# alshai/Big-BWT

Hardware: NVIDIA B200
Metric: pfp_parse_throughput (higher is better)
Workload: dtype u8/u32/u64 integer

## Files before the change

### big-bwt_b200/csrc/pfp_api.cu

```cuda
#include "pfp_common.cuh"
#include "pfp_stages.cuh"
#include <errno.h>
#include <fcntl.h>
#include <stdlib.h>
#include <sys/stat.h>
#include <time.h>
#include <unistd.h>

extern "C" {
int pfp_io_read_file(const char *path, int gz_ok, uint8_t **buf, uint64_t *n, char *err, size_t errlen);
int pfp_io_write_outputs(const char *path, const pfpb200_opts *opts, const pfpb200_outputs *o,
                         char *err, size_t errlen);
}

static double wall_sec() {
    struct timespec ts;
    clock_gettime(CLOCK_MONOTONIC, &ts);
    return (double)ts.tv_sec + 1e-9 * (double)ts.tv_nsec;
}

__global__ void set_u64_k(u64 *p, u64 v) { *p = v; }

__global__ void __launch_bounds__(256) first_invalid_k(const u8 *__restrict__ t, u64 n,
                                                       unsigned long long *__restrict__ first) {
// ... 16 lines not shown

int pfp_first_invalid(pfpb200_ctx *ctx, const u8 *d_text, u64 n, u64 *d_first) {
    if (n == 0) return PFPB200_OK;
    first_invalid_k<<<ctx->sm_count * 8, 256, 0, ctx->stream>>>(d_text, n,
                                                               reinterpret_cast<unsigned long long *>(d_first));
    PFP_LAUNCHED(ctx);
    return PFPB200_OK;
}

extern "C" int pfpb200_abi_version(void) { return PFPB200_ABI_VERSION; }

extern "C" const char *pfpb200_strerror(int code) {
    switch (code) {
        case PFPB200_OK: return "ok";
        case PFPB200_E_ARG: return "invalid argument";
        case PFPB200_E_IO: return "file I/O error";
        case PFPB200_E_CUDA: return "CUDA error (no usable GPU or kernel failure)";
        case PFPB200_E_NOMEM: return "out of memory";
        case PFPB200_E_LIMIT: return "algorithm limit exceeded";
        case PFPB200_E_COLLISION: return "fingerprint collision";
        case PFPB200_E_INTERNAL: return "internal error";
        default: return "unknown error";
    }
}

extern "C" uint32_t pfpb200_launch_count(const pfpb200_ctx *ctx) { return ctx ? ctx->launches : 0; }

extern "C" const char *pfpb200_last_error(const pfpb200_ctx *ctx) { return ctx ? ctx->err : ""; }

static u64 splitmix64(u64 &s) {
    u64 z = (s += 0x9E3779B97F4A7C15ULL);
    z = (z ^ (z >> 30)) * 0xBF58476D1CE4E5B9ULL;
    z = (z ^ (z >> 27)) * 0x94D049BB133111EBULL;
    return z ^ (z >> 31);
}

extern "C" int pfpb200_create(int device, pfpb200_ctx **out) {
    if (!out) return PFPB200_E_ARG;
    *out = nullptr;
    int ndev = 0;
    if (cudaGetDeviceCount(&ndev) != cudaSuccess || device < 0 || device >= ndev) {
        cudaGetLastError();
        return PFPB200_E_CUDA;
    }
    pfpb200_ctx *ctx = new (std::nothrow) pfpb200_ctx();
    if (!ctx) return PFPB200_E_NOMEM;
    ctx->device = device;
    { const char *ev = getenv("PFPB200_LEGACY_K2"); ctx->legacy_k2 = ev && atoi(ev) != 0; }
    { const char *ev = getenv("PFPB200_K1"); ctx->k1_mode = (ev && strcmp(ev, "rolling") == 0) ? 1 : (ev && strcmp(ev, "table") == 0) ? 2 : 0; }
    { const char *ev = getenv("PFPB200_TEST_WEAK_FP"); ctx->weak_fp = (ev && atoi(ev) != 0) ? 1u : 0u; }
    { const char *ev = getenv("PFPB200_NO_SCAN_ALPHA"); ctx->no_scan_alpha = ev && atoi(ev) != 0; }
    { const char *ev = getenv("PFPB200_RANK_FULL_SORT"); ctx->rank_full_sort = ev && atoi(ev) != 0; }
    { const char *ev = getenv("PFPB200_RANK_CHUNK_PASSES"); ctx->rank_chunk_passes = ev && atoi(ev) != 0; }
    { const char *ev = getenv("PFPB200_POOL_BY_WORD"); ctx->pool_by_word = ev && atoi(ev) != 0; }
    { const char *ev = getenv("PFPB200_FUSE_K3"); ctx->fuse_k3 = ev && atoi(ev) != 0; }
    { const char *ev = getenv("PFPB200_TABLE_SCALE"); if (ev && atof(ev) >= 1.2) ctx->table_scale = atof(ev); }
    { const char *ev = getenv("PFPB200_K1_MIX"); ctx->k1_mix = ev ? atoi(ev) : 0; }
    { const char *ev = getenv("PFPB200_K2_WINDOW"); ctx->k2_window = ev ? atoi(ev) : 0; }
    auto bail = [&](int code) { pfpb200_destroy(ctx); return code; };
    if (cudaSetDevice(device) != cudaSuccess) return bail(PFPB200_E_CUDA);
    cudaDeviceProp prop;
    if (cudaGetDeviceProperties(&prop, device) != cudaSuccess) return bail(PFPB200_E_CUDA);
    ctx->sm_count = prop.multiProcessorCount;
    if (cudaStreamCreateWithFlags(&ctx->own_stream, cudaStreamNonBlocking) != cudaSuccess)
        return bail(PFPB200_E_CUDA);
    ctx->stream = ctx->own_stream;
    if (cudaMalloc(&ctx->d_flags, PFP_FLAG_SLOTS * sizeof(u64)) != cudaSuccess ||
        cudaMallocHost(&ctx->h_flags, PFP_FLAG_SLOTS * sizeof(u64)) != cudaSuccess ||
        cudaMalloc(&ctx->d_keys, NH_KEY_WORDS * sizeof(u32)) != cudaSuccess ||
        cudaMalloc(&ctx->d_alpha, 8 * sizeof(u32)) != cudaSuccess)
        return bail(PFPB200_E_NOMEM);
    u32 hk[NH_KEY_WORDS];
    u64 seed = 0x5bd1e9955bd1e995ULL;
    for (u32 i = 0; i < NH_KEY_WORDS; i++) hk[i] = (u32)(splitmix64(seed) >> 32);
    if (cudaMemcpy(ctx->d_keys, hk, sizeof(hk), cudaMemcpyHostToDevice) != cudaSuccess ||
        cudaMemset(ctx->d_flags, 0, PFP_FLAG_SLOTS * sizeof(u64)) != cudaSuccess)
        return bail(PFPB200_E_CUDA);
    set_u64_k<<<1, 1, 0, ctx->stream>>>(&ctx->d_flags[15], 1);
    if (cudaGetLastError() != cudaSuccess || cudaStreamSynchronize(ctx->stream) != cudaSuccess)
        return bail(PFPB200_E_CUDA);
    if (cudaStreamCreateWithFlags(&ctx->aux_stream, cudaStreamNonBlocking) != cudaSuccess ||
        cudaEventCreateWithFlags(&ctx->ev_aux0, cudaEventDisableTiming) != cudaSuccess ||
        cudaEventCreateWithFlags(&ctx->ev_aux1, cudaEventDisableTiming) != cudaSuccess)
        return bail(PFPB200_E_CUDA);
    if (pfp_scan_init(ctx) || pfp_stream_init(ctx) || pfp_phrase_init(ctx) || pfp_prims_init(ctx) ||
        pfp_rank_init(ctx))
        return bail(PFPB200_E_CUDA);
    *out = ctx;
    return PFPB200_OK;
}

extern "C" void pfpb200_destroy(pfpb200_ctx *ctx) {
    if (!ctx) return;
    cudaSetDevice(ctx->device);
    if (ctx->stream) cudaStreamSynchronize(ctx->stream);
    pfp_release_scratch(ctx);
    pfp_release_held(ctx);
    pfp_arena_destroy(ctx);
    if (ctx->own_stream) { cudaStreamSynchronize(ctx->own_stream); cudaStreamDestroy(ctx->own_stream); }
    if (ctx->d_flags) cudaFree(ctx->d_flags);
    if (ctx->h_flags) cudaFreeHost(ctx->h_flags);
    if (ctx->d_keys) cudaFree(ctx->d_keys);
    if (ctx->dna_table) cudaFree(ctx->dna_table);
    if (ctx->iv_etab) cudaFree(ctx->iv_etab);
    if (ctx->iv_xtab) cudaFree(ctx->iv_xtab);
    if (ctx->d_alpha) cudaFree(ctx->d_alpha);
// ... 866 lines not shown
```

### big-bwt_b200/csrc/pfp_common.cuh

```cuda
#pragma once
#include <cuda_runtime.h>
#include <stdint.h>
#include <stdio.h>
#include <string.h>
#include <vector>
#include "pfp_arith.h"
#include "../../include/pfpb200.h"

typedef uint64_t u64;
typedef uint32_t u32;
typedef uint16_t u16;
typedef uint8_t u8;
typedef int64_t i64;

struct PfpBlock { char *p; size_t n; };
struct PfpArena {
    std::vector<PfpBlock> slabs;
    std::vector<PfpBlock> free_list;
    std::vector<PfpBlock> used;
    size_t in_use = 0, peak = 0, total = 0;
};

constexpr int PFP_TILE_T = 256;
constexpr int PFP_TILE_RUN = 128;
constexpr int PFP_TILE = PFP_TILE_T * PFP_TILE_RUN;
struct ScanBits {
    const uint4 *A;
    u64 q_end;
    u64 pos_bias;
    u32 ntiles;
    uint4 *mask;
    u32 *tile_cnt;
    u64 *tile_off;
    u64 total;
    u32 max_tile_cnt;
};

constexpr int PFP_IO_THREADS = 4;
constexpr size_t PFP_IO_CHUNK = (size_t)8 << 20;
struct PfpIo {
    bool ready = false;
    void *slot[PFP_IO_THREADS][2] = {{nullptr}};
    cudaEvent_t ev[PFP_IO_THREADS][2] = {{nullptr}};
    cudaStream_t stream[PFP_IO_THREADS] = {nullptr};
};

struct pfpb200_ctx {
    int device = 0;
    PfpIo io;
    PfpArena arena;
    int sm_count = 148;
    cudaStream_t own_stream = nullptr;
    cudaStream_t stream = nullptr;
    u32 launches = 0;
    int k1_mode = 0;
    u32 *d_alpha = nullptr;
    bool alpha_valid = false;
    u32 *dna_table = nullptr;
    u32 dna_w = 0, dna_p = 0;
    void *iv_etab = nullptr;
    void *iv_xtab = nullptr;
    u32 iv_w = 0, iv_p = 0, iv_cthr = 0;
    int iv_skip = 0;
    bool no_scan_alpha = false;
    bool rank_full_sort = false;
    bool rank_chunk_passes = false;
    bool pool_by_word = false;
    bool fuse_k3 = false;
    double pool_ratio = 0.0;
    bool legacy_k2 = false;
    double table_scale = 2.0;
    u32 weak_fp = 0;
    int k1_mix = 0;
    int k2_window = 0;
    double dedup_ratio = 0.0;
    char err[512] = {0};
    std::vector<void *> scratch;
    std::vector<void *> held;
    void *bp_out[3] = {nullptr, nullptr, nullptr};
    void *up_out = nullptr;
    void *pb_out[4] = {nullptr, nullptr, nullptr, nullptr};
    void *pin_buf[5] = {nullptr, nullptr, nullptr, nullptr, nullptr};
    size_t pin_cap[5] = {0, 0, 0, 0, 0};
    cudaStream_t aux_stream = nullptr;
    cudaEvent_t ev_aux0 = nullptr, ev_aux1 = nullptr;
    cudaStream_t copy_stream = nullptr;
    cudaEvent_t ev_k2 = nullptr, ev_copy = nullptr;
    bool early_copy = false;
    bool early_done = false;
    u32 *d_keys = nullptr;
    u64 *d_flags = nullptr;
    u64 *h_flags = nullptr;
    struct {
        u64 n_in = 0, d = 0, sum_len = 0;
        u32 max_len = 0;
        u32 *uid_of_entry = nullptr, *rep = nullptr, *count = nullptr, *ulen = nullptr, *uwords = nullptr;
        u64 *uoff = nullptr;
        const u32 *len_in = nullptr, *uwords_in = nullptr;
    } mg;
    struct {
        pfpb200_shard desc;
        pfpb200_opts opts;
        u64 *ends = nullptr;
        bool ends_emitted = true;
        ScanBits bits;
        u64 n_trig = 0, P = 0, d = 0;
        u32 *uid = nullptr;
        u64 *wfpa = nullptr, *wfpb = nullptr, *pool = nullptr, *uoff = nullptr, pool_words = 0;
        u32 *ulen = nullptr, *count = nullptr, *uwords = nullptr;
        u32 *route_perm = nullptr;
        u64 *route_ooff = nullptr;
        u64 route_words_to[PFPB200_MAX_RANKS] = {0}, route_pool_to[PFPB200_MAX_RANKS] = {0};
    } sh;
};

#define PFP_FLAG_SLOTS 16
#define PFP_ERRBIT_COLLISION 1ull
#define PFP_ERRBIT_LIMIT 2ull
#define PFP_ERRBIT_INTERNAL 4ull
// ... 104 lines not shown
```

### big-bwt_b200/csrc/pfp_rank.cu

```cuda
#include "pfp_common.cuh"
#include "pfp_stages.cuh"

__device__ __forceinline__ u64 bswap64(u64 v) {
    u32 lo = (u32)v, hi = (u32)(v >> 32);
    return ((u64)__byte_perm(lo, 0, 0x0123) << 32) | (u64)__byte_perm(hi, 0, 0x0123);
}

__device__ __forceinline__ u64 word_key(const u64 *__restrict__ pool, const u64 *__restrict__ uoff,
                                        const u32 *__restrict__ uwords, u32 u, u32 r) {
    return (r < uwords[u]) ? bswap64(__ldg(pool + uoff[u] + r)) : 0ull;
}

struct AlphaMap {
    u32 bits;
    u32 chars;
    u32 depth0;
    u32 pad;
    u8 lut[256];
};

constexpr u32 ALPHA_PROBE_WORDS = 3;

__global__ void alpha_presence_k(const u64 *__restrict__ pool, const u64 *__restrict__ uoff,
                                 const u32 *__restrict__ ulen, u64 d, u32 *__restrict__ gmask) {
// ... 52 lines not shown
                             const u32 *__restrict__ ulen, const u32 *__restrict__ count, u64 d,
                             const AlphaMap *__restrict__ am, u64 *__restrict__ keys, u32 *__restrict__ vals,
                             WordMeta *__restrict__ meta) {
    __shared__ u8 lut[256];
    __shared__ u32 s_bits, s_chars;
    lut[threadIdx.x & 255] = am->lut[threadIdx.x & 255];
    if (threadIdx.x == 0) { s_bits = am->bits; s_chars = am->chars; }
    __syncthreads();
    u64 u = (u64)blockIdx.x * blockDim.x + threadIdx.x;
    if (u >= d) return;
    const u32 bits = s_bits, chars = s_chars, len = ulen[u];
    const u64 off = uoff[u];
    {
        WordMeta wm;
        wm.off = off; wm.len = len; wm.count = count[u];
        meta[u] = wm;
    }
    const u32 nc = len < chars ? len : chars;
    u64 key = 0;
    u64 v = 0;
    for (u32 i = 0; i < nc; i++) {
        if ((i & 7) == 0) v = __ldg(pool + off + (i >> 3));
        u32 c = (u32)(v >> (8 * (i & 7))) & 255u;
        key |= (u64)lut[c] << (64 - bits * (i + 1));
    }
    keys[u] = key;
    vals[u] = (u32)u;
}

__global__ void rank_heads0_k(const u64 *__restrict__ ks, u64 d, const AlphaMap *__restrict__ am, u32 begin_bit,
                              u8 *__restrict__ head, u32 *__restrict__ depth) {
    u64 i = (u64)blockIdx.x * blockDim.x + threadIdx.x;
    if (i >= d) return;
    head[i] = (i == 0 || (ks[i] >> begin_bit) != (ks[i - 1] >> begin_bit)) ? 1 : 0;
    const u32 chars = (64u - begin_bit) / am->bits;
    const u32 d0 = chars / 8u;
    depth[i] = d0 < am->depth0 ? d0 : am->depth0;
}

constexpr u32 LOCAL_MAX = 2048;
constexpr u32 WARP_MAX = 32;

__global__ void groups_compact_k(const u8 *__restrict__ head, const u32 *__restrict__ hscan, u64 d,
                                 const u32 *__restrict__ nheads, u32 *__restrict__ hp,
                                 u32 *__restrict__ gid) {
    u64 i = (u64)blockIdx.x * blockDim.x + threadIdx.x;
    if (i >= d) return;
    u32 g = hscan[i] + head[i] - 1;
    gid[i] = g;
    if (head[i]) hp[g] = (u32)i;
    if (i == 0) hp[*nheads] = (u32)d;
}

__global__ void rank_active_k(const u8 *__restrict__ head, const u32 *__restrict__ gid,
                              const u32 *__restrict__ hp, u64 d, u8 *__restrict__ act,
                              u8 *__restrict__ gh) {
    u64 i = (u64)blockIdx.x * blockDim.x + threadIdx.x;
    if (i >= d) return;
    u32 g = gid[i];
    bool big = (hp[g + 1] - hp[g]) > LOCAL_MAX;
    act[i] = big ? 1 : 0;
    gh[i] = (big && head[i]) ? 1 : 0;
}

__global__ void rank_compact_k(const u8 *__restrict__ act, const u8 *__restrict__ gh,
                               const u32 *__restrict__ ascan, const u32 *__restrict__ gscan,
                               const u32 *__restrict__ ord, const u32 *__restrict__ gid,
                               const u32 *__restrict__ hp, const u32 *__restrict__ depth, u64 d,
                               const u64 *pool, const u64 *uoff, const u32 *uwords,
                               u32 *__restrict__ apos, u64 *__restrict__ keys, u32 *__restrict__ vals,
                               u32 *__restrict__ gid_of_u) {
    u64 i = (u64)blockIdx.x * blockDim.x + threadIdx.x;
    if (i >= d || !act[i]) return;
    u32 j = ascan[i];
    u32 u = ord[i];
    u32 r = depth[hp[gid[i]]];
    apos[j] = (u32)i;
    keys[j] = word_key(pool, uoff, uwords, u, r);
    vals[j] = u;
    gid_of_u[u] = gscan[i] + gh[i] - 1;
}

__global__ void rank_gidkeys_k(const u32 *__restrict__ vs, const u32 *__restrict__ gid_of_u, u64 m,
                               u64 *__restrict__ keys2) {
    u64 j = (u64)blockIdx.x * blockDim.x + threadIdx.x;
    if (j < m) keys2[j] = gid_of_u[vs[j]];
}

__global__ void rank_writeback_k(const u32 *__restrict__ apos, const u64 *__restrict__ gk,
                                 const u32 *__restrict__ vs, u64 m, const u32 *__restrict__ gid,
                                 const u32 *__restrict__ hp, const u32 *__restrict__ depth_in,
                                 const u64 *pool, const u64 *uoff, const u32 *uwords,
                                 u32 *__restrict__ ord, u8 *__restrict__ head,
                                 u32 *__restrict__ depth_out) {
    u64 j = (u64)blockIdx.x * blockDim.x + threadIdx.x;
    if (j >= m) return;
    u32 i = apos[j];
    u32 u = vs[j];
    u32 r = depth_in[hp[gid[i]]];
    ord[i] = u;
    bool newhead = false;
    if (j > 0 && gk[j] == gk[j - 1]) {
        u32 up = vs[j - 1];
        newhead = word_key(pool, uoff, uwords, u, r) != word_key(pool, uoff, uwords, up, r);
        if (newhead) head[i] = 1;
    }
    if (newhead || head[i]) depth_out[i] = r + 1;
}

__device__ __forceinline__ u32 warp_refine(const u64 *__restrict__ wptr, u32 wn, u32 lo, u32 sz, u32 r,
                                           u32 max_chunks, u64 *__restrict__ flags) {
    u64 k0 = 0, k1 = 0, k2 = 0, k3 = 0;
    u32 have = 0;
    for (;;) {
        const bool active = sz > 1;
// ... 200 lines not shown
                if (p + 1 == S.hi[cur][p]) S.tot[l] = incl[e];
            }
        }
        tie_sync<NT>();
#pragma unroll
        for (u32 e = 0; e < TIE_E; e++) {
            const u32 p = p0 + e;
            if (e < E && p < m) {
                const u32 l = S.lo[cur][p], h = S.hi[cur][p], r = S.dep[cur][p];
                u32 np = p, nlo = l, nhi = h, nr = r;
                if (h - l > 1) {
                    const u64 T = S.tot[l];
                    const u32 n0 = (u32)(T & 0xFFFFu), n1 = (u32)((T >> 16) & 0xFFFFu);
                    const u32 idx = (u32)((incl[e] >> (16 * cls[e])) & 0xFFFFu) - 1u;
                    if (cls[e] == 0) { nlo = l; nhi = l + n0; }
                    else if (cls[e] == 1) { nlo = l + n0; nhi = l + n0 + n1; nr = r + 1; }
                    else { nlo = l + n0 + n1; nhi = h; }
                    np = nlo + idx;
                }
                S.uid[cur ^ 1][np] = S.uid[cur][p];
                S.off[cur ^ 1][np] = S.off[cur][p];
                S.wn[cur ^ 1][np] = S.wn[cur][p];
                S.lo[cur ^ 1][np] = (u16)nlo;
                S.hi[cur ^ 1][np] = (u16)nhi;
                S.dep[cur ^ 1][np] = nr;
            }
        }
        tie_sync<NT>();
        cur ^= 1;
    }
    tie_sync<NT>();
    for (u32 i = t; i < m; i += NT) ord[s + i] = S.uid[cur][i];
}

template <int NT, u32 CAP>
__device__ __forceinline__ void tie_refine(TieSort<CAP> &S, u64 *sm_v, u32 *sm_f, u32 t, u32 s, u32 m, u32 r0,
                                           const u64 *pool, const u64 *uoff, const u32 *uwords, u32 max_chunks,
                                           u32 *__restrict__ ord, u64 *__restrict__ flags) {
    const u32 E = (m + NT - 1) / NT;
    if (E <= 2) tie_refine_e<NT, CAP, 2>(S, sm_v, sm_f, t, s, m, r0, pool, uoff, uwords, max_chunks, ord, flags);
    else if (E <= 4) tie_refine_e<NT, CAP, 4>(S, sm_v, sm_f, t, s, m, r0, pool, uoff, uwords, max_chunks, ord, flags);
    else tie_refine_e<NT, CAP, 8>(S, sm_v, sm_f, t, s, m, r0, pool, uoff, uwords, max_chunks, ord, flags);
}

__global__ void rank_lists_k(const u32 *__restrict__ hp, const u32 *__restrict__ nheads, u64 d,
                             u32 *__restrict__ mid_list, u32 *__restrict__ big_list,
                             u32 *__restrict__ warp_list,
                             u32 *__restrict__ counts ) {
    u64 g = (u64)blockIdx.x * blockDim.x + threadIdx.x;
    if (g >= d || g >= *nheads) return;
    const u32 s = hp[g], m = hp[g + 1] - s;
    if (m < 2) return;
    if (m <= WARP_MAX) {
        if ((s >> 5) != ((s + m - 1) >> 5)) warp_list[atomicAdd(&counts[2], 1u)] = (u32)g;
    } else if (m <= MID_MAX) mid_list[atomicAdd(&counts[0], 1u)] = (u32)g;
    else if (m <= LOCAL_MAX) big_list[atomicAdd(&counts[1], 1u)] = (u32)g;
}

__global__ void __launch_bounds__(256) rank_mid_k(const u32 *__restrict__ hp,
                                                  const u32 *__restrict__ list,
                                                  const u32 *__restrict__ count,
                                                  const u32 *__restrict__ depth,
                                                  const u64 *pool, const u64 *uoff, const u32 *uwords,
                                                  u32 max_chunks, u32 *__restrict__ ord,
                                                  u64 *__restrict__ flags) {
    extern __shared__ __align__(16) unsigned char mid_raw[];
    const u32 lane = threadIdx.x & 31, wp = threadIdx.x >> 5;
    TieSort<MID_MAX> &S = reinterpret_cast<TieSort<MID_MAX> *>(mid_raw)[wp];
    u64 *sm_v = nullptr;
    u32 *sm_f = nullptr;
    const u32 n = *count;
    for (u32 q = blockIdx.x * 8 + wp; q < n; q += gridDim.x * 8) {
        const u32 g = list[q];
        const u32 s = hp[g], m = hp[g + 1] - s;
        tie_refine<32, MID_MAX>(S, sm_v, sm_f, lane, s, m, depth[s], pool, uoff, uwords, max_chunks, ord, flags);
    }
}

constexpr u32 LCP_MAX = 256;
constexpr u32 LCP_WALK = 4;
constexpr u32 LCP_HEAD = 1u << 20;
constexpr u32 LCP_MAX_CHUNKS = LCP_HEAD - 1;

template <u32 CAP>
struct LcpSort {
    u64 kb[CAP];
    u32 ka[CAP];
    u32 uid[CAP];
    u32 off[CAP];
    u32 wn[CAP];
    u32 dep[CAP];
    u16 lo[CAP];
    u16 pay[CAP];
    unsigned long long best;
};

__device__ __forceinline__ void prefetch_l2(const void *p) { asm volatile("prefetch.global.L2 [%0];" ::"l"(p)); }

__device__ __forceinline__ bool lcp_less(u32 a0, u64 b0, u32 a1, u64 b1) { return a0 < a1 || (a0 == a1 && b0 < b1); }

__device__ __forceinline__ void lcp_cx_shfl(u32 &ka, u64 &kb, u32 &pay, u32 j, bool up, bool lower) {
    const u32 oa = __shfl_xor_sync(0xffffffffu, ka, j);
    const u64 ob = __shfl_xor_sync(0xffffffffu, kb, j);
    const u32 op = __shfl_xor_sync(0xffffffffu, pay, j);
    const bool mine_less = lcp_less(ka, kb, oa, ob);
    const bool keep = (mine_less == lower) == up;
    if (!keep && !(ka == oa && kb == ob)) { ka = oa; kb = ob; pay = op; }
}

// ... 220 lines not shown
                        const u32 c = code < LCP_HEAD ? code : 2u * LCP_HEAD - 1u - code;
                        S.dep[p] = code == LCP_HEAD ? 0u : c + 1;
                    }
                }
            }
            tie_sync<NT>();
            if (t < 32) {
                u32 carry = 0;
                for (u32 b0 = 0; b0 < m; b0 += 32) {
                    const u32 p = b0 + t;
                    const u32 sm = __ballot_sync(0xffffffffu, p < m && S.pay[p] != 0);
                    if (p < m) {
                        const u32 below = sm & (0xFFFFFFFFu >> (31 - t));
                        S.lo[p] = (u16)(below ? b0 + (31 - __clz(below)) : carry);
                    }
                    if (sm) carry = b0 + (31 - __clz(sm));
                }
            }
            tie_sync<NT>();
        }
    }
    tie_sync<NT>();
    for (u32 p = t; p < m; p += NT) ord[s + p] = S.uid[p];
}

__global__ void __launch_bounds__(256, 3) rank_lcp_k(const u32 *__restrict__ hp, const u32 *__restrict__ list,
                                                  const u32 *__restrict__ count, const u32 *__restrict__ depth,
                                                  const u64 *__restrict__ pool, const u64 *__restrict__ uoff,
                                                  const u32 *__restrict__ uwords, const u32 *__restrict__ occ_of_word,
                                                  u32 max_chunks, u32 *__restrict__ ord, u64 *__restrict__ flags) {
    extern __shared__ __align__(16) unsigned char lcp_raw[];
    const u32 lane = threadIdx.x & 31, wp = threadIdx.x >> 5;
    LcpSort<LCP_MAX> &S = reinterpret_cast<LcpSort<LCP_MAX> *>(lcp_raw)[wp];
    const u32 n = *count;
    for (u32 gq = blockIdx.x * 8 + wp; gq < n; gq += gridDim.x * 8) {
        const u32 g = list[gq];
        const u32 s = hp[g], m = hp[g + 1] - s;
        lcp_refine<32, LCP_MAX>(S, lane, s, m, depth[s], pool, uoff, uwords, occ_of_word, max_chunks, ord, flags);
    }
}

__global__ void __launch_bounds__(256) rank_lcp_cta_k(const u32 *__restrict__ hp, const u32 *__restrict__ list,
                                                      const u32 *__restrict__ count, const u32 *__restrict__ depth,
                                                      const u64 *__restrict__ pool, const u64 *__restrict__ uoff,
                                                      const u32 *__restrict__ uwords, const u32 *__restrict__ occ_of_word,
                                                      u32 max_chunks, u32 *__restrict__ ord, u64 *__restrict__ flags) {
    extern __shared__ __align__(16) unsigned char lcp_cta_raw[];
    LcpSort<LOCAL_MAX> &S = *reinterpret_cast<LcpSort<LOCAL_MAX> *>(lcp_cta_raw);
    const u32 n = *count;
    for (u32 gq = blockIdx.x; gq < n; gq += gridDim.x) {
        const u32 g = list[gq];
        const u32 s = hp[g], m = hp[g + 1] - s;
        lcp_refine<256, LOCAL_MAX>(S, threadIdx.x, s, m, depth[s], pool, uoff, uwords, occ_of_word, max_chunks, ord, flags);
    }
}

__global__ void __launch_bounds__(256) rank_cta_k(const u32 *__restrict__ hp,
                                                  const u32 *__restrict__ list,
                                                  const u32 *__restrict__ count,
                                                  const u32 *__restrict__ depth,
                                                  const u64 *pool, const u64 *uoff, const u32 *uwords,
                                                  u32 max_chunks, u32 *__restrict__ ord,
                                                  u64 *__restrict__ flags) {
    extern __shared__ __align__(16) unsigned char cta_raw[];
    TieSort<LOCAL_MAX> &S = *reinterpret_cast<TieSort<LOCAL_MAX> *>(cta_raw);
    __shared__ u64 sm_v[8];
    __shared__ u32 sm_f[8];
    const u32 n = *count;
    for (u32 q = blockIdx.x; q < n; q += gridDim.x) {
        const u32 g = list[q];
        const u32 s = hp[g], m = hp[g + 1] - s;
        tie_refine<256, LOCAL_MAX>(S, sm_v, sm_f, threadIdx.x, s, m, depth[s], pool, uoff, uwords, max_chunks, ord,
                                   flags);
    }
}

int pfp_rank_init(pfpb200_ctx *ctx) {
    PFP_CUDA(ctx, cudaFuncSetAttribute(rank_cta_k, cudaFuncAttributeMaxDynamicSharedMemorySize,
                                       (int)sizeof(TieSort<LOCAL_MAX>)));
    PFP_CUDA(ctx, cudaFuncSetAttribute(rank_mid_k, cudaFuncAttributeMaxDynamicSharedMemorySize,
                                       (int)(8 * sizeof(TieSort<MID_MAX>))));
    PFP_CUDA(ctx, cudaFuncSetAttribute(rank_lcp_k, cudaFuncAttributeMaxDynamicSharedMemorySize,
                                       (int)(8 * sizeof(LcpSort<LCP_MAX>))));
    PFP_CUDA(ctx, cudaFuncSetAttribute(rank_lcp_cta_k, cudaFuncAttributeMaxDynamicSharedMemorySize,
                                       (int)sizeof(LcpSort<LOCAL_MAX>)));
    return PFPB200_OK;
}

int pfp_rank_stage(pfpb200_ctx *ctx, DictArrays &D, u32 **order, u32 *rounds, bool alpha_from_scan) {
    const int TB = 256;
    const u64 d = D.d;
    const u32 nbd = pfp_blocks(d, TB);
    const u32 max_chunks = (D.max_len + 7) / 8 + 1;
    u64 *k0 = nullptr, *k1 = nullptr, *ks = nullptr;
    u32 *v0 = nullptr, *v1 = nullptr, *vs = nullptr;
    u32 *ord = nullptr, *depth = nullptr, *hscan = nullptr, *hp = nullptr, *gid = nullptr;
    u8 *head = nullptr;
    AlphaMap *am = nullptr;
    u32 *amask = nullptr;
    PFP_TRY(pfp_alloc_t(ctx, &k0, d));
    PFP_TRY(pfp_alloc_t(ctx, &k1, d));
    PFP_TRY(pfp_alloc_t(ctx, &v0, d));
    PFP_TRY(pfp_alloc_t(ctx, &v1, d));
    PFP_TRY(pfp_alloc_t(ctx, &ord, d));
    PFP_TRY(pfp_alloc_t(ctx, &depth, d));
    PFP_TRY(pfp_alloc_t(ctx, &hscan, d));
    PFP_TRY(pfp_alloc_t(ctx, &hp, d + 1));
    PFP_TRY(pfp_alloc_t(ctx, &gid, d));
    PFP_TRY(pfp_alloc_t(ctx, &head, d));
    PFP_TRY(pfp_alloc_t(ctx, &am, 1));
    PFP_TRY(pfp_alloc_t(ctx, &amask, 8));
    if (alpha_from_scan) {
        PFP_CUDA(ctx, cudaMemcpyAsync(amask, ctx->d_alpha, 8 * sizeof(u32), cudaMemcpyDeviceToDevice, ctx->stream));
    } else {
        PFP_CUDA(ctx, cudaMemsetAsync(amask, 0, 8 * sizeof(u32), ctx->stream));
        alpha_presence_k<<<nbd, TB, 0, ctx->stream>>>(D.pool, D.uoff, D.ulen, d, amask);
        PFP_LAUNCHED(ctx);
    }
    alpha_build_k<<<1, 32, 0, ctx->stream>>>(amask, am, alpha_from_scan ? 1 : 0);
    PFP_LAUNCHED(ctx);
    PFP_TRY(pfp_alloc_t(ctx, &D.meta, d));
    rank_keys0_k<<<nbd, TB, 0, ctx->stream>>>(D.pool, D.uoff, D.ulen, D.count, d, am, k0, v0, D.meta);
    PFP_LAUNCHED(ctx);
    int lg = 1;
    while (lg < 32 && (1ull << lg) < d) lg++;
    int sort_bits = (2 * lg + 2 + 7) / 8 * 8;
    if (sort_bits > 64 || ctx->rank_full_sort) sort_bits = 64;
    const int begin_bit = 64 - sort_bits;
    PFP_TRY(pfp_radix_sort_pairs(ctx, k0, v0, k1, v1, d, begin_bit, 64, &ks, &vs));
    rank_heads0_k<<<nbd, TB, 0, ctx->stream>>>(ks, d, am, (u32)begin_bit, head, depth);
    PFP_LAUNCHED(ctx);
    PFP_CUDA(ctx, cudaMemcpyAsync(ord, vs, d * sizeof(u32), cudaMemcpyDeviceToDevice, ctx->stream));

    u8 *act = nullptr, *gh = nullptr;
    u32 *ascan = nullptr, *gscan = nullptr, *apos = nullptr, *gid_of_u = nullptr, *depth2 = nullptr;
    u32 *d_nheads = reinterpret_cast<u32 *>(&ctx->d_flags[4]);
    u32 r = 1;
    bool big_bufs = false;
    for (;; r++) {
        PFP_CUDA(ctx, cudaMemsetAsync(&ctx->d_flags[1], 0, 4 * sizeof(u64), ctx->stream));
        PFP_TRY(pfp_exclusive_scan_u8_u32(ctx, head, hscan, d, d_nheads));
        groups_compact_k<<<nbd, TB, 0, ctx->stream>>>(head, hscan, d, d_nheads, hp, gid);
        PFP_LAUNCHED(ctx);
        if (d < 2) break;
        if (!big_bufs) {
            PFP_TRY(pfp_alloc_t(ctx, &act, d));
            PFP_TRY(pfp_alloc_t(ctx, &gh, d));
            PFP_TRY(pfp_alloc_t(ctx, &ascan, d));
            PFP_TRY(pfp_alloc_t(ctx, &gscan, d));
            big_bufs = true;
        }
        rank_active_k<<<nbd, TB, 0, ctx->stream>>>(head, gid, hp, d, act, gh);
        PFP_LAUNCHED(ctx);
        PFP_TRY(pfp_exclusive_scan_u8_u32(ctx, act, ascan, d, reinterpret_cast<u32 *>(&ctx->d_flags[1])));
        PFP_TRY(pfp_exclusive_scan_u8_u32(ctx, gh, gscan, d, reinterpret_cast<u32 *>(&ctx->d_flags[2])));
        PFP_CUDA(ctx, cudaMemcpyAsync(ctx->h_flags, ctx->d_flags, 3 * sizeof(u64),
                                      cudaMemcpyDeviceToHost, ctx->stream));
        PFP_CUDA(ctx, cudaStreamSynchronize(ctx->stream));
        u64 m = (u32)ctx->h_flags[1], ng = (u32)ctx->h_flags[2];
        if (m == 0) break;
        if (r > max_chunks + 1)
            return pfp_fail(ctx, PFPB200_E_INTERNAL,
                            "ranking did not separate %llu words after %u rounds (duplicate words?)",
                            (unsigned long long)m, r);
        if (!apos) {
            PFP_TRY(pfp_alloc_t(ctx, &apos, d));
            PFP_TRY(pfp_alloc_t(ctx, &gid_of_u, d));
            PFP_TRY(pfp_alloc_t(ctx, &depth2, d));
        }
        rank_compact_k<<<nbd, TB, 0, ctx->stream>>>(act, gh, ascan, gscan, ord, gid, hp, depth, d, D.pool,
                                                    D.uoff, D.uwords, apos, k0, v0, gid_of_u);
        PFP_LAUNCHED(ctx);
        PFP_TRY(pfp_radix_sort_pairs(ctx, k0, v0, k1, v1, m, 0, 64, &ks, &vs));
        u64 *g_in = (ks == k0) ? k1 : k0;
        u32 *v_other = (vs == v0) ? v1 : v0;
        const u32 nbm = pfp_blocks(m, TB);
        rank_gidkeys_k<<<nbm, TB, 0, ctx->stream>>>(vs, gid_of_u, m, g_in);
        PFP_LAUNCHED(ctx);
        int bits = 1;
        while (bits < 32 && (1ull << bits) < ng) bits++;
        u64 *gs = nullptr;
        u32 *vs2 = nullptr;
        PFP_TRY(pfp_radix_sort_pairs(ctx, g_in, vs, ks, v_other, m, 0, bits, &gs, &vs2));
        PFP_CUDA(ctx, cudaMemcpyAsync(depth2, depth, d * sizeof(u32), cudaMemcpyDeviceToDevice, ctx->stream));
        rank_writeback_k<<<nbm, TB, 0, ctx->stream>>>(apos, gs, vs2, m, gid, hp, depth, D.pool, D.uoff,
                                                      D.uwords, ord, head, depth2);
        PFP_LAUNCHED(ctx);
        u32 *tdp = depth; depth = depth2; depth2 = tdp;
    }
    if (d >= 2) {
        u32 *mid_list = v1, *big_list = v0;
        u32 *warp_list = reinterpret_cast<u32 *>(k1);
        u32 *counts = reinterpret_cast<u32 *>(&ctx->d_flags[5]);
        PFP_CUDA(ctx, cudaMemsetAsync(counts, 0, 4 * sizeof(u32), ctx->stream));
        rank_lists_k<<<nbd, TB, 0, ctx->stream>>>(hp, d_nheads, d, mid_list, big_list, warp_list, counts);
        PFP_LAUNCHED(ctx);
        u64 want = (d / 2 + 7) / 8;
        u64 maxb = (u64)ctx->sm_count * 16;
        u32 nbw = (u32)(want < maxb ? want : maxb);
        if (nbw == 0) nbw = 1;
        rank_window_k<<<nbw, 256, 0, ctx->stream>>>(hp, gid, depth, D.pool, D.uoff, D.uwords, d, max_chunks, 0, ord,
                                                    ctx->d_flags);
        PFP_LAUNCHED(ctx);
        rank_warp_k<<<nbw, 256, 0, ctx->stream>>>(hp, warp_list, counts + 2, depth, D.pool, D.uoff, D.uwords, max_chunks,
                                                  ord, ctx->d_flags);
        PFP_LAUNCHED(ctx);
        const bool chunk_passes = ctx->rank_chunk_passes || max_chunks >= LCP_MAX_CHUNKS;
        if (chunk_passes)
            rank_mid_k<<<ctx->sm_count * 4, 256, 8 * sizeof(TieSort<MID_MAX>), ctx->stream>>>(
                hp, mid_list, counts, depth, D.pool, D.uoff, D.uwords, max_chunks, ord, ctx->d_flags);
        else
            rank_lcp_k<<<ctx->sm_count * 6, 256, 8 * sizeof(LcpSort<LCP_MAX>), ctx->stream>>>(
                hp, mid_list, counts, depth, D.pool, D.uoff, D.uwords, D.count, max_chunks, ord, ctx->d_flags);
        PFP_LAUNCHED(ctx);
        if (chunk_passes)
            rank_cta_k<<<ctx->sm_count * 4, 256, sizeof(TieSort<LOCAL_MAX>), ctx->stream>>>(
                hp, big_list, counts + 1, depth, D.pool, D.uoff, D.uwords, max_chunks, ord, ctx->d_flags);
        else
            rank_lcp_cta_k<<<ctx->sm_count * 3, 256, sizeof(LcpSort<LOCAL_MAX>), ctx->stream>>>(
                hp, big_list, counts + 1, depth, D.pool, D.uoff, D.uwords, D.count, max_chunks, ord, ctx->d_flags);
        PFP_LAUNCHED(ctx);
        PFP_CUDA(ctx, cudaMemcpyAsync(ctx->h_flags, ctx->d_flags, sizeof(u64), cudaMemcpyDeviceToHost,
                                      ctx->stream));
        PFP_CUDA(ctx, cudaStreamSynchronize(ctx->stream));
        if (ctx->h_flags[0] & PFP_ERRBIT_INTERNAL)
            return pfp_fail(ctx, PFPB200_E_INTERNAL, "ranking found words that never differ (duplicates?)");
    }
    *rounds = r;
    *order = ord;
    void *to_free[] = {k0, k1, v0, v1, depth, depth2, hscan, hp, gid, head, am, amask, act, gh, ascan,
                       gscan, apos, gid_of_u};
    for (void *q : to_free) PFP_TRY(pfp_free_now(ctx, q));
    return PFPB200_OK;
}

__device__ __forceinline__ void out_span(const u64 *pool, u64 off, u32 len, u32 strip_w, u32 *skip,
                                         u32 *outlen) {
    *skip = 0;
    *outlen = len;
    if (strip_w) {
        u32 l = len - strip_w;
        if ((u8)(pool[off] & 0xFF) == PFP_DOLLAR) { *skip = 1; l -= 1; }
        *outlen = l;
    }
}

__global__ void dict_layout_k(const u32 *__restrict__ ord, u64 d, const DictArrays D, u32 strip_w,
                              u32 *__restrict__ rank_of_uid, u32 *__restrict__ occ,
                              u32 *__restrict__ dl) {
    u64 i = (u64)blockIdx.x * blockDim.x + threadIdx.x;
    if (i >= d) return;
    u32 u = ord[i];
    rank_of_uid[u] = (u32)i + 1;
    const uint4 mv = __ldg(reinterpret_cast<const uint4 *>(D.meta + u));
    occ[i] = mv.w;
    u32 skip, outlen;
    out_span(D.pool, ((u64)mv.y << 32) | mv.x, mv.z, strip_w, &skip, &outlen);
    dl[i] = outlen + 1;
}

constexpr int DC_T = 256;
constexpr int DC_GROUP = 8;

__global__ void __launch_bounds__(DC_T) dict_copy_k(const u32 *__restrict__ ord,
                                                    const u64 *__restrict__ doff, u64 d,
                                                    const DictArrays D, u32 strip_w, u64 total,
                                                    u8 *__restrict__ dict) {
    const u32 li = threadIdx.x & (DC_GROUP - 1);
    if (blockIdx.x == 0 && threadIdx.x == 0) dict[total] = (u8)PFP_END_OF_DICT;
    for (u64 i = (u64)blockIdx.x * (DC_T / DC_GROUP) + (threadIdx.x / DC_GROUP); i < d;
         i += (u64)gridDim.x * (DC_T / DC_GROUP)) {
        const u32 u = ord[i];
        u32 skip, outlen;
        const uint4 mv = __ldg(reinterpret_cast<const uint4 *>(D.meta + u));
        const u64 off = ((u64)mv.y << 32) | mv.x;
        out_span(D.pool, off, mv.z, strip_w, &skip, &outlen);
        const u64 *src64 = D.pool + off;
        const u8 *src = reinterpret_cast<const u8 *>(src64) + skip;
        u8 *dst = dict + doff[i];
// ... 420 lines not shown
```

Baseline: 485.2.

## Resolve small rank groups every round and add a warp-level LCP small-group ranker

Moves the small- and mid-group resolution passes inside the radix refinement loop. Groups of size up to LOCAL_MAX are now finished each round and marked as heads, so later rounds only re-sort the remaining large groups, and the loop exits once no large groups remain. It also adds rank_small_lcp_k, a warp-per-32-window LCP-based ranker that replaces the window-plus-warp kernel pair by default. The trade-off is extra launches and a host sync on every round, plus new, complex per-warp ranking logic that could be wrong.

```diff
diff --git a/big-bwt_b200/csrc/pfp_api.cu b/big-bwt_b200/csrc/pfp_api.cu
--- a/big-bwt_b200/csrc/pfp_api.cu
+++ b/big-bwt_b200/csrc/pfp_api.cu
@@ -92,6 +92,7 @@
     { const char *ev = getenv("PFPB200_NO_SCAN_ALPHA"); ctx->no_scan_alpha = ev && atoi(ev) != 0; }
     { const char *ev = getenv("PFPB200_RANK_FULL_SORT"); ctx->rank_full_sort = ev && atoi(ev) != 0; }
     { const char *ev = getenv("PFPB200_RANK_CHUNK_PASSES"); ctx->rank_chunk_passes = ev && atoi(ev) != 0; }
+    { const char *ev = getenv("PFPB200_RANK_WARP_PASSES"); ctx->rank_warp_passes = ev && atoi(ev) != 0; }
     { const char *ev = getenv("PFPB200_POOL_BY_WORD"); ctx->pool_by_word = ev && atoi(ev) != 0; }
     { const char *ev = getenv("PFPB200_FUSE_K3"); ctx->fuse_k3 = ev && atoi(ev) != 0; }
     { const char *ev = getenv("PFPB200_TABLE_SCALE"); if (ev && atof(ev) >= 1.2) ctx->table_scale = atof(ev); }
diff --git a/big-bwt_b200/csrc/pfp_common.cuh b/big-bwt_b200/csrc/pfp_common.cuh
--- a/big-bwt_b200/csrc/pfp_common.cuh
+++ b/big-bwt_b200/csrc/pfp_common.cuh
@@ -65,6 +65,7 @@
     bool no_scan_alpha = false;
     bool rank_full_sort = false;
     bool rank_chunk_passes = false;
+    bool rank_warp_passes = false;
     bool pool_by_word = false;
     bool fuse_k3 = false;
     double pool_ratio = 0.0;
diff --git a/big-bwt_b200/csrc/pfp_rank.cu b/big-bwt_b200/csrc/pfp_rank.cu
--- a/big-bwt_b200/csrc/pfp_rank.cu
+++ b/big-bwt_b200/csrc/pfp_rank.cu
@@ -128,7 +128,7 @@
     if (i == 0) hp[*nheads] = (u32)d;
 }
 
-__global__ void rank_active_k(const u8 *__restrict__ head, const u32 *__restrict__ gid,
+__global__ void rank_active_k(u8 *__restrict__ head, const u32 *__restrict__ gid,
                               const u32 *__restrict__ hp, u64 d, u8 *__restrict__ act,
                               u8 *__restrict__ gh) {
     u64 i = (u64)blockIdx.x * blockDim.x + threadIdx.x;
@@ -137,6 +137,7 @@
     bool big = (hp[g + 1] - hp[g]) > LOCAL_MAX;
     act[i] = big ? 1 : 0;
     gh[i] = (big && head[i]) ? 1 : 0;
+    if (!big) head[i] = 1;
 }
 
 __global__ void rank_compact_k(const u8 *__restrict__ act, const u8 *__restrict__ gh,
@@ -443,9 +444,10 @@
     const u32 s = hp[g], m = hp[g + 1] - s;
     if (m < 2) return;
     if (m <= WARP_MAX) {
-        if ((s >> 5) != ((s + m - 1) >> 5)) warp_list[atomicAdd(&counts[2], 1u)] = (u32)g;
+        if (warp_list && (s >> 5) != ((s + m - 1) >> 5)) warp_list[atomicAdd(&counts[2], 1u)] = (u32)g;
     } else if (m <= MID_MAX) mid_list[atomicAdd(&counts[0], 1u)] = (u32)g;
     else if (m <= LOCAL_MAX) big_list[atomicAdd(&counts[1], 1u)] = (u32)g;
+    else counts[3] = 1u;
 }
 
 __global__ void __launch_bounds__(256) rank_mid_k(const u32 *__restrict__ hp,
@@ -772,6 +774,153 @@
         const u32 g = list[gq];
         const u32 s = hp[g], m = hp[g + 1] - s;
         lcp_refine<256, LOCAL_MAX>(S, threadIdx.x, s, m, depth[s], pool, uoff, uwords, occ_of_word, max_chunks, ord, flags);
+    }
+}
+
+constexpr u32 SMALL_WALK = 4;
+
+__device__ __forceinline__ u32 small_walk(const u64 *mine, u32 wm, const u64 *head, u32 wh, u32 c, u32 max_chunks,
+                                          u64 &v, u64 &h, bool &bad) {
+    constexpr u32 NC = 2 * SMALL_WALK;
+    for (;;) {
+        const u32 sa = (u32)((uintptr_t)(mine + c) >> 3) & 1u, sb = (u32)((uintptr_t)(head + c) >> 3) & 1u;
+        const ulonglong2 *A = reinterpret_cast<const ulonglong2 *>(mine + c - sa);
+        const ulonglong2 *B = reinterpret_cast<const ulonglong2 *>(head + c - sb);
+        u64 a[NC], b[NC];
+#pragma unroll
+        for (u32 i = 0; i < SMALL_WALK; i++) {
+            ulonglong2 x = make_ulonglong2(0ull, 0ull), y = make_ulonglong2(0ull, 0ull);
+            if (c + 2 * i < wm + sa) x = __ldg(A + i);
+            if (c + 2 * i < wh + sb) y = __ldg(B + i);
+            a[2 * i] = x.x; a[2 * i + 1] = x.y;
+            b[2 * i] = y.x; b[2 * i + 1] = y.y;
+        }
+        const u32 n = NC - (sa | sb);
+        bool found = false;
+#pragma unroll
+        for (u32 i = 0; i < NC; i++) {
+            u64 x = (i + 1 < NC && sa) ? a[i + 1] : a[i];
+            u64 y = (i + 1 < NC && sb) ? b[i + 1] : b[i];
+            if (c + i >= wm) x = 0ull;
+            if (c + i >= wh) y = 0ull;
+            if (!found && i < n && x != y) { found = true; v = bswap64(x); h = bswap64(y); c += i; }
+        }
+        if (found) return c;
+        c += n;
+        if (c >= max_chunks) { bad = true; return c; }
+    }
+}
+
+__global__ void __launch_bounds__(256, 4) rank_small_lcp_k(const u32 *__restrict__ hp, const u32 *__restrict__ gid,
+                                                           const u32 *__restrict__ depth, const u64 *__restrict__ pool,
+                                                           const u64 *__restrict__ uoff, const u32 *__restrict__ uwords,
+                                                           const u32 *__restrict__ occ_of_word, u64 d, u32 max_chunks,
+                                                           u32 *__restrict__ ord, u64 *__restrict__ flags) {
+    __shared__ const u64 *s_ptr[8][64];
+    __shared__ u32 s_wn[8][64];
+    __shared__ u32 s_uid[8][64];
+    __shared__ u32 s_hkey[8][64];
+    __shared__ u32 s_best[8][64];
+    __shared__ u32 s_ka[8][64];
+    __shared__ u64 s_kb[8][64];
+    const u32 lane = threadIdx.x & 31, wp = threadIdx.x >> 5;
+    const u64 nwin = (d + 31) / 32;
+    const u64 nwarps = (u64)gridDim.x * 8;
+    for (u64 k = (u64)blockIdx.x * 8 + wp; k < nwin; k += nwarps) {
+        const u64 w0 = k * 32;
+        u32 s = 0, m = 0;
+        if (w0 + lane < d) {
+            const u32 g = gid[w0 + lane];
+            s = hp[g];
+            m = hp[g + 1] - s;
+        }
+        const bool in0 = m >= 2 && m <= WARP_MAX && s >= w0;
+        const u32 end31 = __shfl_sync(0xffffffffu, in0 ? s + m : 0u, 31);
+        const bool in1 = (u64)end31 > w0 + 32 + lane;
+        if (!__any_sync(0xffffffffu, in0)) continue;
+        const u32 s31 = __shfl_sync(0xffffffffu, s, 31), m31 = __shfl_sync(0xffffffffu, m, 31);
+        u32 pos[2], lo[2], sz[2], dep[2];
+#pragma unroll
+        for (u32 e = 0; e < 2; e++) {
+            const bool in = e ? in1 : in0;
+            const u32 gs = e ? s31 : s, gm = e ? m31 : m;
+            pos[e] = 32 * e + lane;
+            s_uid[wp][pos[e]] = in ? ord[w0 + pos[e]] : 0u;
+            lo[e] = in ? (u32)(gs - w0) : pos[e];
+            sz[e] = in ? gm : 1u;
+            dep[e] = in ? depth[gs] : 0u;
+        }
+#pragma unroll
+        for (u32 e = 0; e < 2; e++) {
+            const bool in = sz[e] > 1;
+            const u32 u = s_uid[wp][pos[e]];
+            const u32 c = in ? occ_of_word[u] : 0u;
+            s_hkey[wp][pos[e]] = ((c < (1u << 26) ? c : (1u << 26) - 1) << 6) | pos[e];
+            if (in) {
+                s_ptr[wp][pos[e]] = pool + uoff[u];
+                s_wn[wp][pos[e]] = uwords[u];
+            }
+        }
+        for (;;) {
+            const bool act0 = sz[0] > 1, act1 = sz[1] > 1;
+            if (!__any_sync(0xffffffffu, act0 || act1)) break;
+            if (act0 && pos[0] == lo[0]) s_best[wp][lo[0]] = 0;
+            if (act1 && pos[1] == lo[1]) s_best[wp][lo[1]] = 0;
+            __syncwarp();
+            if (act0) atomicMax(&s_best[wp][lo[0]], s_hkey[wp][lane]);
+            if (act1) atomicMax(&s_best[wp][lo[1]], s_hkey[wp][32 + lane]);
+            __syncwarp();
+            bool bad = false;
+#pragma unroll 1
+            for (u32 e = 0; e < 2; e++) {
+                const u32 esz = e ? sz[1] : sz[0], elo = e ? lo[1] : lo[0], epos = e ? pos[1] : pos[0];
+                if (esz > 1) {
+                    const u32 hid = s_best[wp][elo] & 63u, me = 32 * e + lane;
+                    u32 code = LCP_HEAD;
+                    u64 v = 0, h = 0;
+                    if (hid != me) {
+                        const u32 c = small_walk(s_ptr[wp][me], s_wn[wp][me], s_ptr[wp][hid], s_wn[wp][hid],
+                                                 e ? dep[1] : dep[0], max_chunks, v, h, bad);
+                        code = v < h ? c : 2u * LCP_HEAD - 1u - c;
+                    }
+                    s_ka[wp][epos] = code;
+                    s_kb[wp][epos] = v;
+                }
+            }
+            if (__any_sync(0xffffffffu, bad)) {
+                if (lane == 0) atomicOr((unsigned long long *)&flags[0], PFP_ERRBIT_INTERNAL);
+                break;
+            }
+            __syncwarp();
+            u32 nlo[2], nsz[2], npos[2];
+#pragma unroll
+            for (u32 e = 0; e < 2; e++) {
+                nlo[e] = lo[e]; nsz[e] = sz[e]; npos[e] = pos[e];
+                if (sz[e] > 1) {
+                    const u32 code = s_ka[wp][pos[e]];
+                    const u64 kv = s_kb[wp][pos[e]];
+                    u32 less = 0, eq = 0, eq_before = 0;
+                    for (u32 q = lo[e]; q < lo[e] + sz[e]; q++) {
+                        const u32 a1 = s_ka[wp][q];
+                        const u64 b1 = s_kb[wp][q];
+                        const bool same = a1 == code && b1 == kv;
+                        less += lcp_less(a1, b1, code, kv) ? 1u : 0u;
+                        eq += same ? 1u : 0u;
+                        eq_before += (same && q < pos[e]) ? 1u : 0u;
+                    }
+                    nlo[e] = lo[e] + less;
+                    nsz[e] = eq;
+                    npos[e] = nlo[e] + eq_before;
+                    if (code != LCP_HEAD) dep[e] = (code < LCP_HEAD ? code : 2u * LCP_HEAD - 1u - code) + 1;
+                }
+            }
+            __syncwarp();
+#pragma unroll
+            for (u32 e = 0; e < 2; e++) { lo[e] = nlo[e]; sz[e] = nsz[e]; pos[e] = npos[e]; }
+        }
+        if (in0) ord[w0 + pos[0]] = s_uid[wp][lane];
+        if (in1) ord[w0 + pos[1]] = s_uid[wp][32 + lane];
+        __syncwarp();
     }
 }
 
@@ -855,6 +1004,8 @@
     u8 *act = nullptr, *gh = nullptr;
     u32 *ascan = nullptr, *gscan = nullptr, *apos = nullptr, *gid_of_u = nullptr, *depth2 = nullptr;
     u32 *d_nheads = reinterpret_cast<u32 *>(&ctx->d_flags[4]);
+    const bool chunk_passes = ctx->rank_chunk_passes || max_chunks >= LCP_MAX_CHUNKS;
+    const bool warp_passes = ctx->rank_warp_passes || max_chunks >= LCP_MAX_CHUNKS;
     u32 r = 1;
     bool big_bufs = false;
     for (;; r++) {
@@ -863,6 +1014,47 @@
         groups_compact_k<<<nbd, TB, 0, ctx->stream>>>(head, hscan, d, d_nheads, hp, gid);
         PFP_LAUNCHED(ctx);
         if (d < 2) break;
+        u32 *mid_list = v1, *big_list = v0;
+        u32 *counts = reinterpret_cast<u32 *>(&ctx->d_flags[5]);
+        PFP_CUDA(ctx, cudaMemsetAsync(counts, 0, 4 * sizeof(u32), ctx->stream));
+        rank_lists_k<<<nbd, TB, 0, ctx->stream>>>(hp, d_nheads, d, mid_list, big_list,
+                                                  warp_passes ? reinterpret_cast<u32 *>(k1) : nullptr, counts);
+        PFP_LAUNCHED(ctx);
+        u64 want = (d / 2 + 7) / 8;
+        u64 maxb = (u64)ctx->sm_count * 16;
+        u32 nbw = (u32)(want < maxb ? want : maxb);
+        if (nbw == 0) nbw = 1;
+        if (warp_passes) {
+            rank_window_k<<<nbw, 256, 0, ctx->stream>>>(hp, gid, depth, D.pool, D.uoff, D.uwords, d, max_chunks, 0,
+                                                        ord, ctx->d_flags);
+            PFP_LAUNCHED(ctx);
+            rank_warp_k<<<nbw, 256, 0, ctx->stream>>>(hp, reinterpret_cast<u32 *>(k1), counts + 2, depth, D.pool,
+                                                      D.uoff, D.uwords, max_chunks, ord, ctx->d_flags);
+        } else {
+            rank_small_lcp_k<<<nbw, 256, 0, ctx->stream>>>(hp, gid, depth, D.pool, D.uoff, D.uwords, D.count, d,
+                                                           max_chunks, ord, ctx->d_flags);
+        }
+        PFP_LAUNCHED(ctx);
+        if (chunk_passes)
+            rank_mid_k<<<ctx->sm_count * 4, 256, 8 * sizeof(TieSort<MID_MAX>), ctx->stream>>>(
+                hp, mid_list, counts, depth, D.pool, D.uoff, D.uwords, max_chunks, ord, ctx->d_flags);
+        else
+            rank_lcp_k<<<ctx->sm_count * 6, 256, 8 * sizeof(LcpSort<LCP_MAX>), ctx->stream>>>(
+                hp, mid_list, counts, depth, D.pool, D.uoff, D.uwords, D.count, max_chunks, ord, ctx->d_flags);
+        PFP_LAUNCHED(ctx);
+        if (chunk_passes)
+            rank_cta_k<<<ctx->sm_count * 4, 256, sizeof(TieSort<LOCAL_MAX>), ctx->stream>>>(
+                hp, big_list, counts + 1, depth, D.pool, D.uoff, D.uwords, max_chunks, ord, ctx->d_flags);
+        else
+            rank_lcp_cta_k<<<ctx->sm_count * 3, 256, sizeof(LcpSort<LOCAL_MAX>), ctx->stream>>>(
+                hp, big_list, counts + 1, depth, D.pool, D.uoff, D.uwords, D.count, max_chunks, ord, ctx->d_flags);
+        PFP_LAUNCHED(ctx);
+        PFP_CUDA(ctx, cudaMemcpyAsync(ctx->h_flags, ctx->d_flags, 7 * sizeof(u64), cudaMemcpyDeviceToHost,
+                                      ctx->stream));
+        PFP_CUDA(ctx, cudaStreamSynchronize(ctx->stream));
+        if (ctx->h_flags[0] & PFP_ERRBIT_INTERNAL)
+            return pfp_fail(ctx, PFPB200_E_INTERNAL, "ranking found words that never differ (duplicates?)");
+        if (reinterpret_cast<const u32 *>(&ctx->h_flags[5])[3] == 0) break;
         if (!big_bufs) {
             PFP_TRY(pfp_alloc_t(ctx, &act, d));
             PFP_TRY(pfp_alloc_t(ctx, &gh, d));
@@ -878,7 +1070,6 @@
                                       cudaMemcpyDeviceToHost, ctx->stream));
         PFP_CUDA(ctx, cudaStreamSynchronize(ctx->stream));
         u64 m = (u32)ctx->h_flags[1], ng = (u32)ctx->h_flags[2];
-        if (m == 0) break;
         if (r > max_chunks + 1)
             return pfp_fail(ctx, PFPB200_E_INTERNAL,
                             "ranking did not separate %llu words after %u rounds (duplicate words?)",
@@ -907,44 +1098,6 @@
                                                       D.uwords, ord, head, depth2);
         PFP_LAUNCHED(ctx);
         u32 *tdp = depth; depth = depth2; depth2 = tdp;
-    }
-    if (d >= 2) {
-        u32 *mid_list = v1, *big_list = v0;
-        u32 *warp_list = reinterpret_cast<u32 *>(k1);
-        u32 *counts = reinterpret_cast<u32 *>(&ctx->d_flags[5]);
-        PFP_CUDA(ctx, cudaMemsetAsync(counts, 0, 4 * sizeof(u32), ctx->stream));
-        rank_lists_k<<<nbd, TB, 0, ctx->stream>>>(hp, d_nheads, d, mid_list, big_list, warp_list, counts);
-        PFP_LAUNCHED(ctx);
-        u64 want = (d / 2 + 7) / 8;
-        u64 maxb = (u64)ctx->sm_count * 16;
-        u32 nbw = (u32)(want < maxb ? want : maxb);
-        if (nbw == 0) nbw = 1;
-        rank_window_k<<<nbw, 256, 0, ctx->stream>>>(hp, gid, depth, D.pool, D.uoff, D.uwords, d, max_chunks, 0, ord,
-                                                    ctx->d_flags);
-        PFP_LAUNCHED(ctx);
-        rank_warp_k<<<nbw, 256, 0, ctx->stream>>>(hp, warp_list, counts + 2, depth, D.pool, D.uoff, D.uwords, max_chunks,
-                                                  ord, ctx->d_flags);
-        PFP_LAUNCHED(ctx);
-        const bool chunk_passes = ctx->rank_chunk_passes || max_chunks >= LCP_MAX_CHUNKS;
-        if (chunk_passes)
-            rank_mid_k<<<ctx->sm_count * 4, 256, 8 * sizeof(TieSort<MID_MAX>), ctx->stream>>>(
-                hp, mid_list, counts, depth, D.pool, D.uoff, D.uwords, max_chunks, ord, ctx->d_flags);
-        else
-            rank_lcp_k<<<ctx->sm_count * 6, 256, 8 * sizeof(LcpSort<LCP_MAX>), ctx->stream>>>(
-                hp, mid_list, counts, depth, D.pool, D.uoff, D.uwords, D.count, max_chunks, ord, ctx->d_flags);
-        PFP_LAUNCHED(ctx);
-        if (chunk_passes)
-            rank_cta_k<<<ctx->sm_count * 4, 256, sizeof(TieSort<LOCAL_MAX>), ctx->stream>>>(
-                hp, big_list, counts + 1, depth, D.pool, D.uoff, D.uwords, max_chunks, ord, ctx->d_flags);
-        else
-            rank_lcp_cta_k<<<ctx->sm_count * 3, 256, sizeof(LcpSort<LOCAL_MAX>), ctx->stream>>>(
-                hp, big_list, counts + 1, depth, D.pool, D.uoff, D.uwords, D.count, max_chunks, ord, ctx->d_flags);
-        PFP_LAUNCHED(ctx);
-        PFP_CUDA(ctx, cudaMemcpyAsync(ctx->h_flags, ctx->d_flags, sizeof(u64), cudaMemcpyDeviceToHost,
-                                      ctx->stream));
-        PFP_CUDA(ctx, cudaStreamSynchronize(ctx->stream));
-        if (ctx->h_flags[0] & PFP_ERRBIT_INTERNAL)
-            return pfp_fail(ctx, PFPB200_E_INTERNAL, "ranking found words that never differ (duplicates?)");
     }
     *rounds = r;
     *order = ord;
```

New measurement: 504.7 (median of 6 runs). 1.04x the previous value.
